# argriffing/raoteh

Hardware: AMD Instinct MI355X
Metric: site log-likelihoods/sec (batched tree pruning) (higher is better)
Workload: dtype f64; 1 GPU; c3: 61-state MG94 codon, 64-leaf balanced tree, 10000 sites/GPU, dense f64 leaf likelihood vectors; encoding=dense, sites_per_gpu=10000, sites_total=10000, states=61, leaves=64, edges=126, batches_rotated=3, reduce=none

## Files before the change

### include/raoteh_hip.h

```cpp
#ifndef RAOTEH_HIP_H
#define RAOTEH_HIP_H

#include <stdint.h>

#ifdef __cplusplus
extern "C" {
#endif

#define RT_OK                0
#define RT_ERR_INVALID      -1
#define RT_ERR_HIP          -2
#define RT_ERR_UNSUPPORTED  -3
#define RT_ERR_NOMEM        -4
#define RT_ERR_RCCL         -5
#define RT_ERR_SINGULAR     -6
#define RT_ERR_ZERO_PROB    -7

#define RT_MAX_STATES      128
#define RT_MAX_EXPECT_STATES 64
#define RT_MAX_EXPECT_STEP_STATES 128
#define RT_MAX_EXPM_STATES 128

#define RT_SITE_OK           0
#define RT_SITE_ZERO_PROB    1
// ... 73 lines not shown
            const double *subtree_probability, const double *node_to_distn_array,
            double *joint_distns);

int rt_mjp_esd_expectation_weights(rt_ctx *ctx, int64_t nnodes, int64_t n,
            int64_t nsites, const int64_t *tree_csr_indices,
            const int64_t *tree_csr_indptr, const double *esd_transitions,
            const double *root_distn, const int64_t *state_mask,
            const double *site_weights, double *edge_weights, int32_t *status);

int rt_mjp_esd_expectation_weights_obs(rt_ctx *ctx, int64_t nnodes, int64_t n,
            int64_t nsites, const int64_t *tree_csr_indices,
            const int64_t *tree_csr_indptr, const double *esd_transitions,
            const double *root_distn, int64_t nobs, const int64_t *obs_nodes, int kind,
            const void *data, const double *site_weights, double *edge_weights,
            int32_t *status);

int rt_mjp_frechet_statistics(rt_ctx *ctx, int64_t n, int64_t nedges, const double *Q,
            int64_t nq, const int64_t *q_index, const double *t, const double *W,
            double *dwell, double *trans);


int rt_model_create(rt_ctx *ctx, int64_t nnodes, int64_t n,
            const int64_t *tree_csr_indices, const int64_t *tree_csr_indptr,
            rt_model **model);
int rt_model_destroy(rt_model *model);

int rt_model_set_rates(rt_model *model, const double *Q, int64_t nq,
            const int64_t *node_q, const double *t);
int rt_model_set_rates_spectral(rt_model *model, const double *A, const double *lam,
            const double *B, const double *D, const double *t);
int rt_model_recompute_transitions(rt_model *model);
int rt_model_set_transitions(rt_model *model, const double *esd_transitions);
int rt_model_get_transitions(rt_model *model, double *esd_transitions);
int rt_model_get_expm_info(rt_model *model, int32_t *info );
int rt_model_set_root_distn(rt_model *model, const double *root_distn);

int rt_model_schedule_depth(const rt_model *model);
int rt_model_get_schedule(const rt_model *model, int32_t *ops, int64_t capacity,
            int64_t *nops);
int rt_build_schedule(int64_t nnodes, const int64_t *tree_csr_indices,
            const int64_t *tree_csr_indptr, int32_t *ops ,
            int32_t *depth);
int rt_set_option(const char *key, int64_t value);
int rt_ctx_set_option(rt_ctx *ctx, const char *key, int64_t value);
int rt_jit_source(int64_t nnodes, const int64_t *tree_csr_indices,
            const int64_t *tree_csr_indptr, int64_t n, int64_t nobs,
            const int64_t *obs_nodes, int64_t prefetch, char *buf, int64_t capacity);

int rt_sites_create(rt_model *model, int64_t nsites, int kind, int64_t nobs,
            const int64_t *obs_nodes, const void *data, rt_sites **sites);
int rt_sites_clone(rt_sites *sites, rt_sites **clone);
int rt_sites_jit_wait(rt_sites *sites);
int rt_jit_wait_all(void);
int rt_sites_destroy(rt_sites *sites);
int64_t rt_sites_device_bytes(const rt_sites *sites);
double rt_sites_jit_compile_seconds(const rt_sites *sites);
int rt_debug_jit_global(rt_sites *sites, const char *name, void *dst, int64_t bytes);
const char *rt_sites_kernel_name(const rt_sites *sites);

int rt_prune(rt_model *model, rt_sites *sites);
int rt_step(rt_model *model, rt_sites *sites, int recompute_transitions);
int rt_expect_step(rt_model *model, rt_sites *sites, int recompute_transitions,
            double *dwell, double *root_posterior, double *trans, int32_t *status);
#define RT_MAX_POSTERIOR_SETS 8
int rt_sites_posteriors(rt_model *model, rt_sites *sites, int recompute_transitions,
            int64_t n_node_sets, const uint64_t *node_sets,
// ... 136 lines not shown
```

### raoteh_amd/_lib.py

```python
from __future__ import annotations

import ctypes
import os
from ctypes import (POINTER, c_char_p, c_double, c_int, c_int32,
                    c_int64, c_ubyte, c_void_p)

__all__ = ['HipLibraryError', 'RaotehHipError', 'lib', 'check', 'LIB_PATH']

LIB_PATH = os.environ.get(
    'RAOTEH_HIP_LIB',
    os.path.join(os.path.dirname(os.path.abspath(__file__)), 'libraoteh_hip.so'))

RT_OK = 0
RT_ERR_INVALID = -1
RT_ERR_HIP = -2
RT_ERR_UNSUPPORTED = -3
RT_ERR_NOMEM = -4
RT_ERR_RCCL = -5
RT_ERR_SINGULAR = -6
RT_ERR_ZERO_PROB = -7

RT_OBS_DENSE, RT_OBS_STATE, RT_OBS_MASK = 0, 1, 2
RT_K_EXPM, RT_K_PRUNE, RT_K_REDUCE, RT_K_COMBINE = 0, 1, 2, 3
RT_SITE_ZERO_PROB = 1
# ... 53 lines not shown
    'rt_mcy_esd_get_node_to_pmap': (c_int, [c_void_p, c_int64, c_int64, c_int64,
                                            _p_i64, _p_i64, _p_f64, _p_i64,
                                            _p_f64, _p_f64]),
    'rt_mcy_esd_passes': (c_int, [c_void_p, c_int64, c_int64, c_int64,
                                  _p_i64, _p_i64, _p_f64, _p_i64,
                                  _p_f64, _p_f64]),
    'rt_mc0_esd_get_node_to_distn': (c_int, [c_void_p, c_int64, c_int64, c_int64,
                                             _p_i64, _p_i64, _p_f64, _p_f64,
                                             _p_f64, _p_f64, _p_i32]),
    'rt_mc0_esd_get_joint_endpoint_distn': (c_int, [c_void_p, c_int64, c_int64,
                                                    c_int64, _p_i64, _p_i64,
                                                    _p_f64, _p_f64, _p_f64,
                                                    _p_f64]),
    'rt_mjp_esd_expectation_weights': (c_int, [c_void_p, c_int64, c_int64, c_int64,
                                               _p_i64, _p_i64, _p_f64, _p_f64, _p_i64,
                                               _p_f64, _p_f64, _p_i32]),
    'rt_mjp_esd_expectation_weights_obs': (c_int, [c_void_p, c_int64, c_int64, c_int64,
                                                   _p_i64, _p_i64, _p_f64, _p_f64, c_int64,
                                                   _p_i64, c_int, c_void_p, _p_f64, _p_f64,
                                                   _p_i32]),
    'rt_mjp_frechet_statistics': (c_int, [c_void_p, c_int64, c_int64, _p_f64, c_int64, _p_i64,
                                          _p_f64, _p_f64, _p_f64, _p_f64]),
    'rt_model_create': (c_int, [c_void_p, c_int64, c_int64, _p_i64, _p_i64,
                                POINTER(c_void_p)]),
    'rt_model_destroy': (c_int, [c_void_p]),
    'rt_model_set_rates': (c_int, [c_void_p, _p_f64, c_int64, _p_i64, _p_f64]),
    'rt_model_set_rates_spectral': (c_int, [c_void_p, _p_f64, _p_f64, _p_f64, _p_f64, _p_f64]),
    'rt_expm_spectral': (c_int, [c_void_p, c_int64, c_int64, _p_f64, _p_f64, _p_f64, _p_f64,
                                 _p_f64, _p_f64]),
    'rt_model_recompute_transitions': (c_int, [c_void_p]),
    'rt_model_set_transitions': (c_int, [c_void_p, _p_f64]),
    'rt_model_get_transitions': (c_int, [c_void_p, _p_f64]),
    'rt_model_get_expm_info': (c_int, [c_void_p, _p_i32]),
    'rt_model_set_root_distn': (c_int, [c_void_p, _p_f64]),
    'rt_model_schedule_depth': (c_int, [c_void_p]),
    'rt_model_get_schedule': (c_int, [c_void_p, _p_i32, c_int64, _p_i64]),
    'rt_build_schedule': (c_int, [c_int64, _p_i64, _p_i64, _p_i32, _p_i32]),
    'rt_set_option': (c_int, [c_char_p, c_int64]),
    'rt_ctx_set_option': (c_int, [c_void_p, c_char_p, c_int64]),
    'rt_sites_jit_compile_seconds': (c_double, [c_void_p]),
    'rt_sites_kernel_name': (c_char_p, [c_void_p]),
    'rt_debug_jit_global': (c_int, [c_void_p, c_char_p, c_void_p, c_int64]),
    'rt_jit_source': (c_int, [c_int64, _p_i64, _p_i64, c_int64, c_int64, _p_i64, c_int64,
                              c_char_p, c_int64]),
    'rt_sites_create': (c_int, [c_void_p, c_int64, c_int, c_int64, _p_i64,
                                c_void_p, POINTER(c_void_p)]),
    'rt_sites_clone': (c_int, [c_void_p, POINTER(c_void_p)]),
    'rt_sites_jit_wait': (c_int, [c_void_p]),
    'rt_jit_wait_all': (c_int, []),
    'rt_expect_step': (c_int, [c_void_p, c_void_p, c_int, _p_f64, _p_f64, _p_f64, _p_i32]),
    'rt_sites_posteriors': (c_int, [c_void_p, c_void_p, c_int, c_int64, c_void_p, c_int64,
                                    c_void_p, c_int64, _p_i64, _p_f64, _p_f64, _p_f64, _p_i32]),
    'rt_sites_branch_expectations': (c_int, [c_void_p, c_void_p, c_int, c_int64, _p_f64, _p_f64,
                                             _p_f64, _p_i32]),
    'rt_sites_branch_profiles': (c_int, [c_void_p, c_void_p, c_int, c_int64, _p_f64, _p_f64,
                                         _p_f64, _p_i32]),
    'rt_model_get_branch_lengths': (c_int, [c_void_p, _p_f64]),
    'rt_model_nni_moves': (c_int, [c_void_p, _p_i32, c_int64, _p_i64]),
    'rt_tree_nni_moves': (c_int, [c_int64, _p_i64, _p_i64, _p_i32, c_int64, _p_i64]),
    'rt_sites_nni_scores': (c_int, [c_void_p, c_void_p, c_int, c_int64, _p_f64, _p_f64, _p_f64,
                                    _p_i32]),
    'rt_sites_placements': (c_int, [c_void_p, c_void_p, c_int, c_int64, c_int, c_void_p, c_int64,
                                    _p_f64, c_int64, _p_f64, _p_f64, _p_f64, _p_i32]),
    'rt_model_spr_moves': (c_int, [c_void_p, c_int64, _p_i32, c_int64, _p_i64]),
    'rt_tree_spr_moves': (c_int, [c_int64, _p_i64, _p_i64, c_int64, _p_i32, c_int64, _p_i64]),
    'rt_sites_spr_scores': (c_int, [c_void_p, c_void_p, c_int, c_int64, c_int64, _p_f64, _p_f64,
# ... 105 lines not shown
```

### raoteh_amd/csrc/api.hip

```cpp
#include "common.h"
#include "partition_plan.h"

#include <algorithm>
#include <atomic>
#include <functional>
#include <cmath>
#include <cstdlib>


static thread_local char g_err[512] = "";

void rt_set_error(const char *fmt, ...)
{
    va_list ap;
    va_start(ap, fmt);
    vsnprintf(g_err, sizeof(g_err), fmt, ap);
    va_end(ap);
}

extern "C" const char *rt_last_error(void) { return g_err; }
extern "C" int rt_version(void) { return 100; }

extern "C" int rt_device_count(int *count)
{
// ... 748 lines not shown
    r.nq = nq;
    return rate_sets_run_expm(m);
}

extern "C" int rt_model_recompute_transitions(rt_model *m)
{
    RT_REQUIRE(m, "null model");
    RT_REQUIRE(m->d_Q || m->spectral, "rt_model_set_rates has not been called");
    RT_HIP(hipSetDevice(m->ctx->device));
    return model_run_expm(m);
}

extern "C" int rt_model_set_transitions(rt_model *m, const double *esd)
{
    RT_REQUIRE(m && esd, "null pointer");
    RT_HIP(hipSetDevice(m->ctx->device));
    RT_HIP(hipStreamSynchronize(m->ctx->stream));
    RT_HIP(hipMemcpy(m->d_P, esd, (size_t)m->nnodes * m->n * m->n * 8,
                     hipMemcpyHostToDevice));
    m->have_P = true;
    m->rates_current = false;
    m->frag_dirty = true;
    return rt_launch_pfrag(m);
}

extern "C" int rt_model_get_transitions(rt_model *m, double *esd)
{
    RT_REQUIRE(m && esd, "null pointer");
    RT_REQUIRE(m->have_P, "the model has no transition matrices yet");
    RT_HIP(hipSetDevice(m->ctx->device));
    RT_HIP(hipStreamSynchronize(m->ctx->stream));
    RT_HIP(hipMemcpy(esd, m->d_P, (size_t)m->nnodes * m->n * m->n * 8,
                     hipMemcpyDeviceToHost));
    return RT_OK;
}

extern "C" int rt_model_get_expm_info(rt_model *m, int32_t *info)
{
    RT_REQUIRE(m && info, "null pointer");
    RT_HIP(hipSetDevice(m->ctx->device));
    RT_HIP(hipStreamSynchronize(m->ctx->stream));
    RT_HIP(hipMemcpy(info, m->d_info, (size_t)m->nnodes * 8, hipMemcpyDeviceToHost));
    for (int64_t v = 1; v < m->nnodes; ++v)
        if (info[2 * v] < 0) {
            rt_set_error("expm: the matrix of the edge above node %lld has a non-finite entry or "
                         "norm (Taylor scheme), or its Pade denominator is singular "
                         "(RAOTEH_EXPM=pade)", (long long)v);
            return RT_ERR_SINGULAR;
        }
    return RT_OK;
}

extern "C" int rt_model_set_root_distn(rt_model *m, const double *root_distn)
{
    RT_REQUIRE(m, "null model");
    RT_HIP(hipSetDevice(m->ctx->device));
    std::vector<double> w((size_t)m->n, 1.0);
    if (root_distn) w.assign(root_distn, root_distn + m->n);
    RT_HIP(hipStreamSynchronize(m->ctx->stream));
    RT_HIP(hipMemcpy(m->d_root, w.data(), m->n * 8, hipMemcpyHostToDevice));
    return RT_OK;
}

extern "C" int rt_model_schedule_depth(const rt_model *m)
{
    return m ? m->max_depth : -1;
// ... 1933 lines not shown
```

### raoteh_amd/csrc/common.h

```cpp
#pragma once

#include <hip/hip_runtime.h>
#include <hip/hip_ext.h>

#include <cstdarg>
#include <cstdint>
#include <cstdio>
#include <cstring>
#include <memory>
#include <string>
#include <type_traits>
#include <vector>

#include "../../include/raoteh_hip.h"


void rt_set_error(const char *fmt, ...);

#define RT_HIP(call)                                                          \
    do {                                                                      \
        hipError_t e_ = (call);                                               \
        if (e_ != hipSuccess) {                                               \
            rt_set_error("%s failed: %s (%s:%d)", #call,                      \
                         hipGetErrorString(e_), __FILE__, __LINE__);          \
// ... 61 lines not shown
    char name[64] = "";
};

static const int RT_TOTALS_SLOTS = 4096;

struct rt_ctx {
    int device = 0;
    hipStream_t stream = nullptr;
    int num_cus = 0;
    bool timing = false;
    int timing_period = 1;
    rt_timing_slot slots[RT_K_COUNT];
    hipEvent_t ev_start = nullptr, ev_stop = nullptr;
    double *d_totals_arena = nullptr;
    std::vector<int> totals_free;
    hipEvent_t ev_reduced = nullptr;
    hipEvent_t comm_events[8] = {};
    int comm_event_next = 0;
    unsigned char *d_scratch = nullptr;
    size_t scratch_bytes = 0;
    void *comm = nullptr;
    hipStream_t comm_stream = nullptr;
    void *rccl = nullptr;
    int opt_force_generic = -2;
    int opt_jit = -2;
    int opt_jit_block_sites = -2;
    int opt_jit_async = -2;
    int opt_rescale = -2;
    int opt_leaf_state_kernels = -2;
    struct rt_sites *pending_reduce = nullptr;
    size_t expm_attr_lds = 0;
    size_t expm_ts_attr_lds[8] = {0, 0, 0, 0, 0, 0, 0, 0};
    size_t expm_split_attr_lds = 0;
    size_t expm_w8_attr_lds[3] = {0, 0, 0};
    size_t expm_wide_attr_lds[8] = {0, 0, 0, 0, 0, 0, 0, 0};
    double *d_expm_scratch = nullptr;
    void *expect_cache = nullptr;
    size_t expm_scratch_bytes = 0;
    int live_models = 0, live_chains = 0;
};
static const int RT_OPT_UNSET = -2;

static const int RT_FAST_MAX_DEPTH = 16;

struct rt_op {
    int32_t node;
    int32_t obs;
    int32_t pop;
    int32_t dst;
};

struct rt_rate_sets {
    int64_t K = 0;
    int64_t capacity = 0;
    int64_t nq = 0, q_capacity = 0;
    uint64_t epoch = 0;
    double *d_Q = nullptr;
    int32_t *d_qidx = nullptr;
    double *d_t = nullptr;
    int32_t *d_info = nullptr;
    int32_t *d_step_of_node = nullptr;
    double *d_P = nullptr;
    double *d_Pfrag = nullptr, *d_Pquad = nullptr, *d_Pcol = nullptr;
    int64_t pcol_capacity = 0;
    int64_t P_stride = 0, frag_stride = 0, quad_stride = 0, pcol_stride = 0;
};

// ... 314 lines not shown
```

### raoteh_amd/csrc/expm.hip

```cpp
#include "common.h"

#include <algorithm>
#include "reduce.h"

#include <cstdlib>

namespace {

__constant__ double c_theta[5] = {1.495585217958292e-2, 2.539398330063230e-1,
                                  9.504178996162932e-1, 2.097847961257068e0,
                                  5.371920351148152e0};
__constant__ double c_b3[4] = {120., 60., 12., 1.};
__constant__ double c_b5[6] = {30240., 15120., 3360., 420., 30., 1.};
__constant__ double c_b7[8] = {17297280., 8648640., 1995840., 277200.,
                               25200., 1512., 56., 1.};
__constant__ double c_b9[10] = {17643225600., 8821612800., 2075673600.,
                                302702400., 30270240., 2162160., 110880.,
                                3960., 90., 1.};
__constant__ double c_b13[14] = {64764752532480000., 32382376266240000.,
                                 7771770303897600., 1187353796428800.,
                                 129060195264000., 10559470521600.,
                                 670442572800., 33522128640., 1323241920.,
                                 40840800., 960960., 16380., 182., 1.};

// ... 586 lines not shown
}

template <int NT>
__device__ __forceinline__ void wave8_tiles(int wave, int &m, int &j0, int &nc)
{
    if (NT == 4) { m = wave >> 1; j0 = 2 * (wave & 1); nc = 2; }
    else if (wave < 6) { m = wave / 3; j0 = wave - 3 * m; nc = 1; }
    else { m = 2; j0 = wave == 6 ? 0 : 2; nc = wave == 6 ? 2 : 1; }
}

template <int NT>
__device__ __forceinline__ void load_left8(const double *X, int m, double (&a)[4 * NT])
{
    constexpr int LD = 16 * NT + 1;
    const int lane = threadIdx.x & 63;
    const double *ap = X + (16 * m + (lane & 15)) * LD + (lane >> 4);
#pragma unroll
    for (int kk = 0; kk < 4 * NT; ++kk) a[kk] = ap[4 * kk];
}

template <int NT>
__device__ __forceinline__ void load_tiles8(const double *M, half_tiles &t, int m, int j0, int nc)
{
    constexpr int LD = 16 * NT + 1;
    const int lane = threadIdx.x & 63;
    const int lr = lane & 15, lq = lane >> 4;
#pragma unroll
    for (int v = 0; v < 2; ++v)
#pragma unroll
        for (int r = 0; r < 4; ++r)
            t.v[v][r] = v < nc ? M[(16 * m + 4 * r + lq) * LD + 16 * (j0 + v) + lr] : 0.0;
}

template <int NT, int NC>
__device__ __forceinline__ void mm8(const double (&a)[4 * NT], const double *Y, double *C,
                                    int m, int j0, int nc_wave, bool seed, double c0, double c1,
                                    double c2, double nd, const half_tiles *R1,
                                    const half_tiles *R2, half_tiles *out = nullptr,
                                    const double *top = nullptr, double *C2 = nullptr,
                                    bool fine = false)
{
    RT_FINE(0);
    constexpr int LD = 16 * NT + 1, KS = 4 * NT;
    const int nc = NC ? NC : nc_wave;
    const int lane = threadIdx.x & 63;
    const int lr = lane & 15, lq = lane >> 4;
    const double *bp = Y + lq * LD + 16 * j0 + lr;
    const int o1 = nc > 1 ? 16 : 0;
    double b00 = bp[0], b01 = bp[o1];
    double b10 = bp[4 * LD], b11 = bp[4 * LD + o1];
    double4_t acc[2];
#pragma unroll
    for (int v = 0; v < 2; ++v) {
        acc[v] = (double4_t){0.0, 0.0, 0.0, 0.0};
        if (seed && v < nc) {
            const int col = 16 * (j0 + v) + lr;
#pragma unroll
            for (int r = 0; r < 4; ++r) {
                const int row = 16 * m + 4 * r + lq;
                double w = c1 * R1->v[v][r];
                w = fma(c2, R2->v[v][r], w);
                if (row == col && (double)row < nd) w += c0;
                acc[v][r] = w;
            }
        }
    }
    RT_FINE(1);
#pragma unroll
    for (int kk = 0; kk < KS; ++kk) {
        const int kn = kk + 2 < KS ? kk + 2 : KS - 1;
        const double b20 = bp[4 * kn * LD], b21 = bp[4 * kn * LD + o1];
        __builtin_amdgcn_sched_barrier(0);
        acc[0] = __builtin_amdgcn_mfma_f64_16x16x4f64(a[kk], b00, acc[0], 0, 0, 0);
        if (NC != 1 && nc > 1)
            acc[1] = __builtin_amdgcn_mfma_f64_16x16x4f64(a[kk], b01, acc[1], 0, 0, 0);
        __builtin_amdgcn_sched_barrier(0);
        b00 = b10; b01 = b11;
        b10 = b20; b11 = b21;
    }
    RT_FINE(2);
    if (out) {
#pragma unroll
        for (int v = 0; v < 2; ++v)
#pragma unroll
            for (int r = 0; r < 4; ++r) out->v[v][r] = acc[v][r];
    }
    __syncthreads();
    RT_FINE(3);
#pragma unroll
    for (int v = 0; v < 2; ++v)
        if (v < nc) {
            const int col = 16 * (j0 + v) + lr;
#pragma unroll
            for (int r = 0; r < 4; ++r) {
                const int row = 16 * m + 4 * r + lq;
                C[row * LD + col] = acc[v][r];
                if (top) {
                    double w = top[1] * R1->v[v][r];
                    w = fma(top[2], R2->v[v][r], w);
                    w = fma(top[3], acc[v][r], w);
                    C2[row * LD + col] = w + ((row == col && (double)row < top[4]) ? top[0] : 0.0);
                }
            }
        }
    RT_FINE(4);
    __syncthreads();
    RT_FINE(5);
}

__device__ int rt_expm_trace_on = 0;
__device__ unsigned long long rt_expm_trace[8];
#define RT_EXPM_STAMP(k)                                                              \
    if (trace_on && blockIdx.x == (SPLIT ? 2 : 1) && threadIdx.x == 0)                \
        rt_expm_trace[k] = __builtin_readcyclecounter()

template <int NT, bool GLOBAL, bool SPLIT = false, int WAVES = 4>
__global__ void __launch_bounds__(64 * WAVES)
expm_taylor_kernel(int n, const double *__restrict__ Q, const int *__restrict__ qidx,
                   const double *__restrict__ tt, double *__restrict__ P,
                   int *__restrict__ info, const int *__restrict__ step_of_node,
                   int frag_kind, double *__restrict__ Pfrag, double *__restrict__ Pquad,
                   double *__restrict__ scratch, rt_reduce_args red)
{
    extern __shared__ __attribute__((aligned(16))) unsigned char smem[];
    if (red.partial && blockIdx.x == gridDim.x - 1) {
        rt_reduce_partials_body(red.partial, red.npartials, red.totals, red.nsites);
        return;
    }
    constexpr int RN = 16 * NT;
    constexpr int LD = RN + 1;
    constexpr int MSZ = RN * LD;
    __shared__ double colsum[RN];
    const int trace_on = rt_expm_trace_on;
    RT_EXPM_STAMP(0);
    double *B0 = GLOBAL ? scratch + (size_t)blockIdx.x * 4 * MSZ : (double *)smem;
    double *B1 = B0 + MSZ;
    double *B2 = B1 + MSZ;
    double *B3 = B2 + MSZ;

    static_assert(!SPLIT || (NT == 4 && !GLOBAL), "two workgroups per matrix: 49 <= n <= 64");
    static_assert(WAVES == 4 || (WAVES == 8 && !GLOBAL && (NT == 3 || NT == 4)),
                  "two waves per SIMD: LDS-resident, 33 <= n <= 64");
    constexpr int NTH = 64 * WAVES;
    const int b = SPLIT ? (int)(blockIdx.x >> 1) : (int)blockIdx.x;
    const int half = SPLIT ? (int)(blockIdx.x & 1) : 0;
    const int tid = threadIdx.x;
    const int nn = n * n;
    const int KSn = (n + 3) / 4, NTn = (n + 15) / 16;
    double *Pb = P + (long)b * nn;
    const int qi = qidx[b];
    const int step = step_of_node ? step_of_node[b] : -1;
    constexpr int RP0 = GLOBAL ? 1 : TPB / RN;
    constexpr int PER0 = GLOBAL ? 1 : (RN + RP0 - 1) / RP0;
    double q0[PER0];
    if (!GLOBAL) {
        const int jc = tid % RN, g = tid / RN;
#pragma unroll
        for (int u = 0; u < PER0; ++u) {
            const int i = g + u * RP0;
            q0[u] = (g < RP0 && i < n && jc < n) ? Q[i * n + jc] : 0.0;
        }
    }
    const double t_early = tt[b];
    if (qi < 0) {
        for (int e = tid; e < nn; e += NTH) Pb[e] = 0.0;
        if (info && tid == 0) { info[2 * b] = 0; info[2 * b + 1] = 0; }
        if (step >= 0 && frag_kind == 0)
            for (int e = tid; e < nn; e += NTH) Pfrag[(long)step * nn + e] = 0.0;
        if (step >= 0 && frag_kind == 1) {
            const int total = NTn * ((KSn + 1) / 2) * 128;
            for (int e = tid; e < total; e += NTH) Pfrag[(long)step * total + e] = 0.0;
            if (Pquad)
                for (int e = tid; e < KSn * KSn * 16; e += NTH)
                    Pquad[(long)step * rt_quad_stride(n) + e] = 0.0;
        }
        return;
    }
    const double *Qb = Q + (long)qi * nn;
    const double t = t_early;
    double nrm = 0.0;
    if (!GLOBAL) {
        constexpr int RP = TPB / RN;
        constexpr int PER = (RN + RP - 1) / RP;
        __shared__ double colpart[RP][RN];
        const int jc = tid % RN, g = tid / RN;
        const bool active = g < RP;
        double v[PER];
        double part = 0.0;
        if (qi > 0) {
#pragma unroll
            for (int u = 0; u < PER; ++u) {
                const int i = g + u * RP;
                q0[u] = (active && i < n && jc < n) ? Qb[i * n + jc] : 0.0;
            }
        }
#pragma unroll
        for (int u = 0; u < PER; ++u) v[u] = q0[u] * t;
#pragma unroll
        for (int u = 0; u < PER; ++u) {
            const int i = g + u * RP;
            if (active && i < RN) B0[i * LD + jc] = v[u];
            part += fabs(v[u]);
        }
        if (active) colpart[g][jc] = part;
        __syncthreads();
        if (tid < RN) {
            double sum = 0.0;
#pragma unroll
            for (int r = 0; r < RP; ++r) sum += colpart[r][tid];
            colsum[tid] = sum;
        }
        __syncthreads();
        {
            const int ln = tid & 63;
            nrm = ln < RN ? colsum[ln] : 0.0;
#pragma unroll
            for (int o = 32; o > 0; o >>= 1) nrm = fmax(nrm, __shfl_xor(nrm, o, 64));
        }
    } else {
        constexpr int PER = (MSZ + TPB - 1) / TPB;
        for (int c0 = 0; c0 < PER; c0 += 8) {
            double v[8];
#pragma unroll
            for (int u = 0; u < 8; ++u) {
                const int e = (c0 + u) * TPB + tid;
                const int i = e / LD, jx = e - i * LD;
                v[u] = (e < MSZ && i < n && jx < n) ? Qb[i * n + jx] * t : 0.0;
            }
#pragma unroll
            for (int u = 0; u < 8; ++u) {
                const int e = (c0 + u) * TPB + tid;
                if (e < MSZ) B0[e] = v[u];
            }
        }
        __syncthreads();
        for (int jx = tid; jx < RN; jx += TPB) {
            double sum = 0.0;
            for (int i = 0; i < n; ++i) sum += fabs(B0[i * LD + jx]);
            colsum[jx] = sum;
        }
        __syncthreads();
        for (int jj = 0; jj < RN; ++jj) nrm = fmax(nrm, colsum[jj]);
    }
    RT_EXPM_STAMP(1);
    if (!(nrm < 1e300)) {
        for (int e = tid; e < nn; e += NTH) Pb[e] = __builtin_nan("");
        if (info && tid == 0) { info[2 * b] = -1; info[2 * b + 1] = 0; }
        return;
    }
    int m = 15, s = 0;
    if (nrm <= c_theta_taylor[0]) m = 3;
    else if (nrm <= c_theta_taylor[1]) m = 6;
    else if (nrm <= c_theta_taylor[2]) m = 9;
    else if (nrm <= c_theta_taylor[3]) m = 12;
    else if (nrm > c_theta_taylor[4]) {
        int e;
        const double f = frexp(nrm / c_theta_taylor[4], &e);
        s = (f == 0.5) ? e - 1 : e;
        if (s < 0) s = 0;
    }
    m = __builtin_amdgcn_readfirstlane(m);
    s = __builtin_amdgcn_readfirstlane(s);
    if (info && tid == 0) { info[2 * b] = m; info[2 * b + 1] = s; }
    if (s > 0) {
        const double sc = ldexp(1.0, -s);
        for (int e = tid; e < MSZ; e += NTH) B0[e] *= sc;
        __syncthreads();
    }
    const int q = m / 3;
    RT_EXPM_STAMP(2);
    if constexpr (WAVES == 8) {
        const int wave = __builtin_amdgcn_readfirstlane(tid >> 6);
        int wm, wj, wn;
        wave8_tiles<NT>(wave, wm, wj, wn);
        constexpr int NCF = NT == 4 ? 2 : 0;
        const double nd = (double)n;
        const double tops8[5] = {c_inv_fact[3 * (q - 1)], c_inv_fact[3 * (q - 1) + 1],
                                 c_inv_fact[3 * (q - 1) + 2], c_inv_fact[m], nd};
        double left[4 * NT];
        half_tiles ra, ra2;
        load_left8<NT>(B0, wm, left);
        load_tiles8<NT>(B0, ra, wm, wj, wn);
        mm8<NT, NCF>(left, B0, B1, wm, wj, wn, false, 0.0, 0.0, 0.0, nd, nullptr, nullptr,
                     &ra2);
        mm8<NT, NCF>(left, B1, B2, wm, wj, wn, false, 0.0, 0.0, 0.0, nd, &ra, &ra2, nullptr,
                     tops8, B3);
        RT_EXPM_STAMP(3);
        RT_EXPM_STAMP(4);
        if (q >= 2) load_left8<NT>(B2, wm, left);
        if (SPLIT && s == 0) {
            if constexpr (SPLIT) {
                const int hj = 2 * half + (wave & 1);
                half_tiles ha, ha2;
                load_tiles8<NT>(B0, ha, wm, hj, 1);
                load_tiles8<NT>(B1, ha2, wm, hj, 1);
#pragma unroll
                for (int u = 3; u >= 0; --u)
                    if (u <= q - 2)
                        mm8<NT, 1>(left, B3, B3, wm, hj, 1, true, c_inv_fact[3 * u],
                                   c_inv_fact[3 * u + 1], c_inv_fact[3 * u + 2], nd, &ha, &ha2,
                                   nullptr, nullptr, nullptr,
                                   trace_on && blockIdx.x == 2 && u == 0);
            }
        } else {
            for (int jj = q - 2; jj >= 0; --jj)
                mm8<NT, NCF>(left, B3, B3, wm, wj, wn, true, c_inv_fact[3 * jj],
                             c_inv_fact[3 * jj + 1], c_inv_fact[3 * jj + 2], nd, &ra, &ra2);
        }
        RT_EXPM_STAMP(5);
        for (int r = 0; r < s; ++r) {
            load_left8<NT>(B3, wm, left);
            mm8<NT, NCF>(left, B3, B3, wm, wj, wn, false, 0.0, 0.0, 0.0, nd, nullptr, nullptr);
        }
    } else {
        lane_tiles<NT> ra, ra2;
        load_tiles<NT>(B0, ra);
        mm_blocked<NT>(B0, B0, B1, nullptr, nullptr, nullptr, nullptr, nullptr, &ra2);
        __shared__ double tops[5];
        {
            const int base = 3 * (q - 1);
            if (tid == 0) {
                tops[0] = c_inv_fact[base];
                tops[1] = c_inv_fact[base + 1];
                tops[2] = c_inv_fact[base + 2];
                tops[3] = c_inv_fact[m];
                tops[4] = (double)n;
            }
            __syncthreads();
        }
        mm_blocked<NT>(B0, B1, B2, nullptr, nullptr, nullptr, &ra, &ra2, nullptr, tops, B3);
        RT_EXPM_STAMP(3);
        RT_EXPM_STAMP(4);
        __shared__ double cfs_all[5][4];
        if (tid < 20) cfs_all[tid >> 2][tid & 3] = (tid & 3) == 3 ? (double)n
                                                                 : c_inv_fact[3 * (tid >> 2) + (tid & 3)];
        __syncthreads();
        if (SPLIT && s == 0) {
            if constexpr (SPLIT) {
                half_tiles ha, ha2;
                load_half_tiles(B0, ha, half);
                load_half_tiles(B1, ha2, half);
                double hc[4][3];
#pragma unroll
                for (int u = 0; u < 4; ++u)
#pragma unroll
                    for (int e = 0; e < 3; ++e) hc[u][e] = c_inv_fact[3 * u + e];
                const double nd = (double)n;
#pragma unroll
                for (int u = 3; u >= 0; --u)
                    if (u <= q - 2)
                        mm_half(B2, B3, B3, hc[u][0], hc[u][1], hc[u][2], nd, ha, ha2, half,
                                trace_on && blockIdx.x == 2 && u == 0);
            }
        } else {
            for (int jj = q - 2; jj >= 0; --jj)
                mm_blocked<NT>(B2, B3, B3, cfs_all[jj], B0, B1, &ra, &ra2);
        }
        RT_EXPM_STAMP(5);
        for (int r = 0; r < s; ++r) mm_blocked<NT>(B3, B3, B3, nullptr, nullptr, nullptr);
    }
    RT_EXPM_STAMP(6);

    const double *Xb = B3;
    if constexpr (SPLIT) {
        const int jc = 32 * half + (tid & 31), g = tid >> 5;
        if (jc < n)
            for (int i = g; i < n; i += NTH / 32) Pb[i * n + jc] = Xb[i * LD + jc];
        if (step >= 0 && frag_kind == 1) {
            const int KP = (KSn + 1) / 2;
            const int total = NTn * KP * 128;
            for (int blk = tid >> 7; blk < NTn * 4; blk += NTH >> 7) {
                const int mm = blk >> 2, qq = 4 * half + (blk & 3);
                if (qq < KP) {
                    const int e = (mm * KP + qq) * 128 + (tid & 127);
                    const int e2 = e & 1;
                    const int ln = (e >> 1) & 63;
                    const int row = 16 * mm + (ln & 15);
                    const int col = 4 * (2 * qq + e2) + (ln >> 4);
                    Pfrag[(long)step * total + e] = (col < RN) ? Xb[row * LD + col] : 0.0;
                }
            }
        }
        RT_EXPM_STAMP(7);
        return;
    }
    if (!GLOBAL) {
        constexpr int RP = NTH / RN;
        const int jc = tid % RN, g = tid / RN;
        if (g < RP && jc < n)
            for (int i = g; i < n; i += RP) Pb[i * n + jc] = Xb[i * LD + jc];
    } else {
        for (int e = tid; e < nn; e += TPB) {
            const int i = e / n, j = e - i * n;
            Pb[e] = Xb[i * LD + j];
        }
    }
// ... 320 lines not shown
        const char *wv = getenv("RAOTEH_EXPM_WIDE");
        if (global && !(wv && atoi(wv) == 0) && !d_Pquad) {
            bool split2 = 2 * vcount + extra <= (int64_t)std::max(2, ctx->num_cus);
            if (const char *v = getenv("RAOTEH_EXPM_SPLIT")) split2 = atoi(v) != 0;
            const size_t wgs = (size_t)count * (split2 ? 2 : 1);
            const size_t need = wgs * ((nt + 1) / 2) * 4 * nt * 256 * 8;
            if (need > ctx->expm_scratch_bytes) {
                RT_HIP(hipStreamSynchronize(ctx->stream));
                hipFree(ctx->d_expm_scratch);
                ctx->d_expm_scratch = nullptr;
                ctx->expm_scratch_bytes = 0;
                RT_HIP(hipMalloc((void **)&ctx->d_expm_scratch, need));
                ctx->expm_scratch_bytes = need;
            }
            RT_TRY(rt_expm_wide_launch(ctx, nt, split2, wgs + extra, n, d_Q, d_qidx, d_t, d_P, d_info,
                                       d_step_of_node, frag_kind, d_Pfrag, red));
            return RT_OK;
        }
        hipEvent_t ev = nullptr;
        rt_time_begin(ctx, RT_K_EXPM, global ? "expm_taylor_ps_mfma_global" : "expm_taylor_ps_mfma",
                      &ev);
#define RT_TAYLOR(NTV, GL)                                                                      \
        do {                                                                                    \
            if (lds_t > ctx->expm_ts_attr_lds[NTV - 1]) {                                       \
                RT_HIP(hipFuncSetAttribute((const void *)expm_taylor_kernel<NTV, GL>,           \
                                           hipFuncAttributeMaxDynamicSharedMemorySize,          \
                                           (int)lds_t));                                        \
                ctx->expm_ts_attr_lds[NTV - 1] = lds_t;                                         \
            }                                                                                   \
            RT_LAUNCH_TIMED(ctx, (expm_taylor_kernel<NTV, GL>), dim3((unsigned)count + extra),  \
                            dim3(TPB), lds_t, (int)n, d_Q, d_qidx, d_t, d_P, d_info,            \
                            d_step_of_node, frag_kind, d_Pfrag, d_Pquad, scratch, red);         \
        } while (0)
#define RT_TAYLOR8(NTV, SP, SLOT)                                                               \
        do {                                                                                    \
            if (lds_t > ctx->expm_w8_attr_lds[SLOT]) {                                          \
                RT_HIP(hipFuncSetAttribute((const void *)expm_taylor_kernel<NTV, false, SP, 8>, \
                                           hipFuncAttributeMaxDynamicSharedMemorySize,          \
                                           (int)lds_t));                                        \
                ctx->expm_w8_attr_lds[SLOT] = lds_t;                                            \
            }                                                                                   \
            RT_LAUNCH_TIMED(ctx, (expm_taylor_kernel<NTV, false, SP, 8>),                       \
                            dim3((SP ? 2u : 1u) * (unsigned)count + extra), dim3(512), lds_t,   \
                            (int)n, d_Q, d_qidx, d_t, d_P, d_info, d_step_of_node, frag_kind,   \
                            d_Pfrag, d_Pquad, scratch, red);                                    \
        } while (0)
        const char *wv8 = getenv("RAOTEH_EXPM_WAVES");
        const bool waves8 = (nt == 3 || nt == 4) && !(wv8 && atoi(wv8) == 4);
        bool split2 = nt == 4 && 2 * vcount + extra <= (int64_t)std::max(2, ctx->num_cus) && !d_Pquad;
        if (const char *v = getenv("RAOTEH_EXPM_SPLIT")) split2 = nt == 4 && !d_Pquad && atoi(v) != 0;
        if (split2 && waves8) {
            snprintf(ctx->slots[RT_K_EXPM].name, sizeof(ctx->slots[RT_K_EXPM].name),
                     "expm_taylor_ps_mfma_split2");
            RT_TAYLOR8(4, true, 2);
        } else if (split2) {
            if (lds_t > ctx->expm_split_attr_lds) {
                RT_HIP(hipFuncSetAttribute((const void *)expm_taylor_kernel<4, false, true>,
                                           hipFuncAttributeMaxDynamicSharedMemorySize, (int)lds_t));
                ctx->expm_split_attr_lds = lds_t;
            }
            snprintf(ctx->slots[RT_K_EXPM].name, sizeof(ctx->slots[RT_K_EXPM].name),
                     "expm_taylor_ps_mfma_split2");
            RT_LAUNCH_TIMED(ctx, (expm_taylor_kernel<4, false, true>),
                            dim3(2u * (unsigned)count + extra), dim3(TPB), lds_t, (int)n, d_Q, d_qidx,
                            d_t, d_P, d_info, d_step_of_node, frag_kind, d_Pfrag, d_Pquad, scratch,
                            red);
        } else
        switch (nt) {
        case 1: RT_TAYLOR(1, false); break;
        case 2: RT_TAYLOR(2, false); break;
        case 3: if (waves8) RT_TAYLOR8(3, false, 0); else RT_TAYLOR(3, false); break;
        case 4: if (waves8) RT_TAYLOR8(4, false, 1); else RT_TAYLOR(4, false); break;
        case 5: RT_TAYLOR(5, true); break;
        case 6: RT_TAYLOR(6, true); break;
        case 7: RT_TAYLOR(7, true); break;
        default: RT_TAYLOR(8, true); break;
        }
#undef RT_TAYLOR
#undef RT_TAYLOR8
        RT_HIP(hipGetLastError());
        if (getenv("RAOTEH_EXPM_TRACE")) {
            static int armed = 0;
            unsigned long long tr[8];
            RT_HIP(hipStreamSynchronize(ctx->stream));
            if (armed) {
                RT_HIP(hipMemcpyFromSymbol(tr, HIP_SYMBOL(rt_expm_trace), sizeof tr));
                unsigned long long fn[8];
                RT_HIP(hipMemcpyFromSymbol(fn, HIP_SYMBOL(rt_expm_fine), sizeof fn));
                fprintf(stderr, "[raoteh_amd] last Horner half product: seed + first operands %llu, k loop "
                        "%llu, barrier %llu, write-back %llu, barrier %llu\n", fn[1] - fn[0],
                        fn[2] - fn[1], fn[3] - fn[2], fn[4] - fn[3], fn[5] - fn[4]);
                fprintf(stderr, "[raoteh_amd] expm trace (clocks, workgroup 1): load + norm %llu, order %llu, "
                        "A^2 A^3 %llu, block %llu, Horner %llu, squarings %llu, store %llu; total %llu\n",
                        tr[1] - tr[0], tr[2] - tr[1], tr[3] - tr[2], tr[4] - tr[3], tr[5] - tr[4],
                        tr[6] - tr[5], tr[7] - tr[6], tr[7] - tr[0]);
            }
            const int on = 1;
            RT_HIP(hipMemcpyToSymbol(HIP_SYMBOL(rt_expm_trace_on), &on, sizeof on));
            armed = 1;
        }
        rt_time_end(ctx, RT_K_EXPM, ev);
        return RT_OK;
    }
    hipEvent_t ev = nullptr;
    rt_time_begin(ctx, RT_K_EXPM, "expm_mfma_regsolve", &ev);
    RT_LAUNCH_TIMED(ctx, expm_kernel, dim3((unsigned)count + extra), dim3(TPB), lds,
                       (int)n, d_Q, d_qidx, d_t, d_P, d_info, d_step_of_node, frag_kind,
                       d_Pfrag, d_Pquad, red);
    RT_HIP(hipGetLastError());
    rt_time_end(ctx, RT_K_EXPM, ev);
    return RT_OK;
}
// ... 1 lines not shown
```

### raoteh_amd/device.py

```python
from __future__ import annotations

import atexit
import collections
import ctypes
import weakref
from ctypes import byref, c_char_p, c_double, c_int, c_int32, c_int64, c_void_p

import numpy as np

from . import _lib
from ._tree import TreeArrays

__all__ = ['check_rate_sets', 'check_site_sets', 'Context', 'get_context', 'TreeModel', 'SiteBatch', 'device_count', 'Posteriors',
           'states_to_mask', 'BranchExpectations', 'check_branch_coefs', 'SampledStates', 'SampledMappings',
           'MapStates']

_shutting_down = []
atexit.register(_shutting_down.append, True)

_KINDS = {'dense': _lib.RT_OBS_DENSE, 'state': _lib.RT_OBS_STATE,
          'mask': _lib.RT_OBS_MASK}


def _f64(a):
# ... 763 lines not shown
        A, lam, B = _f64(A), _f64(lam), _f64(B)
        n = self.nstates
        if A.shape != (n, n) or B.shape != (n, n) or lam.shape != (n,):
            raise ValueError('expected the array to be square')
        D = None if D is None else _f64(D)
        if D is not None and D.shape != (n,):
            raise ValueError('D must have one entry per state')
        if t is None:
            t = self.tree.branch_lengths()
        t = _f64(t)
        if t.shape != (self.tree.nnodes,):
            raise ValueError('t must have one entry per node')
        _lib.check(_lib.lib().rt_model_set_rates_spectral(
            self._h, _ptr(A, c_double), _ptr(lam, c_double), _ptr(B, c_double),
            None if D is None else _ptr(D, c_double), _ptr(t, c_double)))
        self._rates = None

    def recompute_transitions(self):
        _lib.check(_lib.lib().rt_model_recompute_transitions(self._h))

    def set_transitions(self, esd):
        esd = _f64(esd)
        if esd.shape != (self.tree.nnodes, self.nstates, self.nstates):
            raise ValueError('esd_transitions has the wrong shape')
        _lib.check(_lib.lib().rt_model_set_transitions(self._h,
                                                       _ptr(esd, c_double)))

    def get_transitions(self):
        esd = np.empty((self.tree.nnodes, self.nstates, self.nstates))
        _lib.check(_lib.lib().rt_model_get_transitions(self._h,
                                                       _ptr(esd, c_double)))
        return esd

    def expm_info(self):
        info = np.zeros((self.tree.nnodes, 2), dtype=np.int32)
        _lib.check(_lib.lib().rt_model_get_expm_info(self._h,
                                                     _ptr(info, c_int32)))
        return info

    def set_root_distn(self, root_distn=None):
        if root_distn is None:
            _lib.check(_lib.lib().rt_model_set_root_distn(self._h, None))
            self._root_w = None
            return
        w = _f64(root_distn)
        if w.shape != (self.nstates,):
            raise ValueError('root shape mismatch: %s %s' % (
                (self.nstates,), w.shape))
        _lib.check(_lib.lib().rt_model_set_root_distn(self._h,
                                                      _ptr(w, c_double)))
        self._root_w = w.copy()

    def upload_sites(self, obs_nodes, data, kind='dense', site_sets=None, nsets=None):
        code = _KINDS[kind]
        idx = _i64([self.tree.node_to_index[v] for v in obs_nodes])
        if kind == 'dense':
            data = _f64(data)
            ok = data.ndim == 3 and data.shape[2] == self.nstates
        elif kind == 'state':
            data = _as_uint8_states(data, self.nstates)
            ok = data.ndim == 2
        else:
            data = np.ascontiguousarray(data, dtype=np.uint64)
            words = (self.nstates + 63) // 64
            ok = (data.ndim == 2 and words == 1) or (data.ndim == 3 and data.shape[2] == words)
        if not ok or data.shape[1] != len(idx):
# ... 539 lines not shown
```

Before: 55.23 million sites/s.

## Add lean eight-wave expm form overlapping norm/order with first product and ping-pong buffers

Adds a LEAN variant of the eight-wave Taylor expm kernel. One wave computes the 1-norm and Taylor order while the others start the first matrix product speculatively, redoing it only when scaling is needed. The Horner and squaring steps now ping-pong between two buffers, which lets mm8 skip the aliasing barrier. It is on by default unless RAOTEH_EXPM_SERIAL=0, and a fragment read-back API is added alongside. The prune-throughput metric only benefits if the expm kernel falls within the timed region.

```diff
diff --git a/include/raoteh_hip.h b/include/raoteh_hip.h
--- a/include/raoteh_hip.h
+++ b/include/raoteh_hip.h
@@ -129,6 +129,7 @@
 int rt_model_recompute_transitions(rt_model *model);
 int rt_model_set_transitions(rt_model *model, const double *esd_transitions);
 int rt_model_get_transitions(rt_model *model, double *esd_transitions);
+int rt_model_get_fragments(rt_model *model, double *frags, int64_t *ndoubles);
 int rt_model_get_expm_info(rt_model *model, int32_t *info );
 int rt_model_set_root_distn(rt_model *model, const double *root_distn);
 
diff --git a/raoteh_amd/_lib.py b/raoteh_amd/_lib.py
--- a/raoteh_amd/_lib.py
+++ b/raoteh_amd/_lib.py
@@ -109,6 +109,7 @@
     'rt_model_set_transitions': (c_int, [c_void_p, _p_f64]),
     'rt_model_get_transitions': (c_int, [c_void_p, _p_f64]),
     'rt_model_get_expm_info': (c_int, [c_void_p, _p_i32]),
+    'rt_model_get_fragments': (c_int, [c_void_p, _p_f64, _p_i64]),
     'rt_model_set_root_distn': (c_int, [c_void_p, _p_f64]),
     'rt_model_schedule_depth': (c_int, [c_void_p]),
     'rt_model_get_schedule': (c_int, [c_void_p, _p_i32, c_int64, _p_i64]),
diff --git a/raoteh_amd/csrc/api.hip b/raoteh_amd/csrc/api.hip
--- a/raoteh_amd/csrc/api.hip
+++ b/raoteh_amd/csrc/api.hip
@@ -804,6 +804,22 @@
     RT_HIP(hipStreamSynchronize(m->ctx->stream));
     RT_HIP(hipMemcpy(esd, m->d_P, (size_t)m->nnodes * m->n * m->n * 8,
                      hipMemcpyDeviceToHost));
+    return RT_OK;
+}
+
+extern "C" int rt_model_get_fragments(rt_model *m, double *frags, int64_t *ndoubles)
+{
+    RT_REQUIRE(m && ndoubles, "null pointer");
+    if (!frags) {
+        *ndoubles = pfrag_doubles(m);
+        return RT_OK;
+    }
+    RT_REQUIRE(m->have_P, "the model has no transition matrices yet");
+    RT_REQUIRE(*ndoubles >= 0 && *ndoubles <= pfrag_doubles(m), "the image has %lld doubles",
+               (long long)pfrag_doubles(m));
+    RT_HIP(hipSetDevice(m->ctx->device));
+    RT_HIP(hipStreamSynchronize(m->ctx->stream));
+    RT_HIP(hipMemcpy(frags, m->d_Pfrag, (size_t)*ndoubles * 8, hipMemcpyDeviceToHost));
     return RT_OK;
 }
 
diff --git a/raoteh_amd/csrc/common.h b/raoteh_amd/csrc/common.h
--- a/raoteh_amd/csrc/common.h
+++ b/raoteh_amd/csrc/common.h
@@ -117,7 +117,7 @@
     size_t expm_attr_lds = 0;
     size_t expm_ts_attr_lds[8] = {0, 0, 0, 0, 0, 0, 0, 0};
     size_t expm_split_attr_lds = 0;
-    size_t expm_w8_attr_lds[3] = {0, 0, 0};
+    size_t expm_w8_attr_lds[6] = {0, 0, 0, 0, 0, 0};
     size_t expm_wide_attr_lds[8] = {0, 0, 0, 0, 0, 0, 0, 0};
     double *d_expm_scratch = nullptr;
     void *expect_cache = nullptr;
diff --git a/raoteh_amd/csrc/expm.hip b/raoteh_amd/csrc/expm.hip
--- a/raoteh_amd/csrc/expm.hip
+++ b/raoteh_amd/csrc/expm.hip
@@ -642,7 +642,7 @@
             t.v[v][r] = v < nc ? M[(16 * m + 4 * r + lq) * LD + 16 * (j0 + v) + lr] : 0.0;
 }
 
-template <int NT, int NC>
+template <int NT, int NC, bool ALIAS = true>
 __device__ __forceinline__ void mm8(const double (&a)[4 * NT], const double *Y, double *C,
                                     int m, int j0, int nc_wave, bool seed, double c0, double c1,
                                     double c2, double nd, const half_tiles *R1,
@@ -695,7 +695,7 @@
 #pragma unroll
             for (int r = 0; r < 4; ++r) out->v[v][r] = acc[v][r];
     }
-    __syncthreads();
+    if (ALIAS) __syncthreads();
     RT_FINE(3);
 #pragma unroll
     for (int v = 0; v < 2; ++v)
@@ -718,13 +718,29 @@
     RT_FINE(5);
 }
 
+__device__ __forceinline__ void taylor_order(double nrm, int &m, int &s)
+{
+    m = 15;
+    s = 0;
+    if (nrm <= c_theta_taylor[0]) m = 3;
+    else if (nrm <= c_theta_taylor[1]) m = 6;
+    else if (nrm <= c_theta_taylor[2]) m = 9;
+    else if (nrm <= c_theta_taylor[3]) m = 12;
+    else if (nrm > c_theta_taylor[4]) {
+        int e;
+        const double f = frexp(nrm / c_theta_taylor[4], &e);
+        s = (f == 0.5) ? e - 1 : e;
+        if (s < 0) s = 0;
+    }
+}
+
 __device__ int rt_expm_trace_on = 0;
 __device__ unsigned long long rt_expm_trace[8];
 #define RT_EXPM_STAMP(k)                                                              \
     if (trace_on && blockIdx.x == (SPLIT ? 2 : 1) && threadIdx.x == 0)                \
         rt_expm_trace[k] = __builtin_readcyclecounter()
 
-template <int NT, bool GLOBAL, bool SPLIT = false, int WAVES = 4>
+template <int NT, bool GLOBAL, bool SPLIT = false, int WAVES = 4, bool LEAN = false>
 __global__ void __launch_bounds__(64 * WAVES)
 expm_taylor_kernel(int n, const double *__restrict__ Q, const int *__restrict__ qidx,
                    const double *__restrict__ tt, double *__restrict__ P,
@@ -751,6 +767,8 @@
     static_assert(!SPLIT || (NT == 4 && !GLOBAL), "two workgroups per matrix: 49 <= n <= 64");
     static_assert(WAVES == 4 || (WAVES == 8 && !GLOBAL && (NT == 3 || NT == 4)),
                   "two waves per SIMD: LDS-resident, 33 <= n <= 64");
+    static_assert(!LEAN || WAVES == 8, "the form with fewer barriers is an eight-wave form");
+    __shared__ int order_lds[2];
     constexpr int NTH = 64 * WAVES;
     const int b = SPLIT ? (int)(blockIdx.x >> 1) : (int)blockIdx.x;
     const int half = SPLIT ? (int)(blockIdx.x & 1) : 0;
@@ -814,6 +832,20 @@
         }
         if (active) colpart[g][jc] = part;
         __syncthreads();
+        if constexpr (LEAN) {
+            if (tid >> 6 == 7) {
+                const int ln = tid & 63;
+                double sum = 0.0;
+#pragma unroll
+                for (int r = 0; r < RP; ++r) sum += colpart[r][ln < RN ? ln : 0];
+                nrm = ln < RN ? sum : 0.0;
+#pragma unroll
+                for (int o = 32; o > 0; o >>= 1) nrm = fmax(nrm, __shfl_xor(nrm, o, 64));
+                int m7 = -1, s7 = 0;
+                if (nrm < 1e300) taylor_order(nrm, m7, s7);
+                if (ln == 0) { order_lds[0] = m7; order_lds[1] = s7; }
+            }
+        } else {
         if (tid < RN) {
             double sum = 0.0;
 #pragma unroll
@@ -826,6 +858,7 @@
             nrm = ln < RN ? colsum[ln] : 0.0;
 #pragma unroll
             for (int o = 32; o > 0; o >>= 1) nrm = fmax(nrm, __shfl_xor(nrm, o, 64));
+        }
         }
     } else {
         constexpr int PER = (MSZ + TPB - 1) / TPB;
@@ -853,22 +886,14 @@
         for (int jj = 0; jj < RN; ++jj) nrm = fmax(nrm, colsum[jj]);
     }
     RT_EXPM_STAMP(1);
+    int m = 15, s = 0;
+    if constexpr (!LEAN) {
     if (!(nrm < 1e300)) {
         for (int e = tid; e < nn; e += NTH) Pb[e] = __builtin_nan("");
         if (info && tid == 0) { info[2 * b] = -1; info[2 * b + 1] = 0; }
         return;
     }
-    int m = 15, s = 0;
-    if (nrm <= c_theta_taylor[0]) m = 3;
-    else if (nrm <= c_theta_taylor[1]) m = 6;
-    else if (nrm <= c_theta_taylor[2]) m = 9;
-    else if (nrm <= c_theta_taylor[3]) m = 12;
-    else if (nrm > c_theta_taylor[4]) {
-        int e;
-        const double f = frexp(nrm / c_theta_taylor[4], &e);
-        s = (f == 0.5) ? e - 1 : e;
-        if (s < 0) s = 0;
-    }
+    taylor_order(nrm, m, s);
     m = __builtin_amdgcn_readfirstlane(m);
     s = __builtin_amdgcn_readfirstlane(s);
     if (info && tid == 0) { info[2 * b] = m; info[2 * b + 1] = s; }
@@ -877,7 +902,9 @@
         for (int e = tid; e < MSZ; e += NTH) B0[e] *= sc;
         __syncthreads();
     }
-    const int q = m / 3;
+    }
+    int q = m / 3;
+    double *last = B3;
     RT_EXPM_STAMP(2);
     if constexpr (WAVES == 8) {
         const int wave = __builtin_amdgcn_readfirstlane(tid >> 6);
@@ -885,19 +912,52 @@
         wave8_tiles<NT>(wave, wm, wj, wn);
         constexpr int NCF = NT == 4 ? 2 : 0;
         const double nd = (double)n;
-        const double tops8[5] = {c_inv_fact[3 * (q - 1)], c_inv_fact[3 * (q - 1) + 1],
-                                 c_inv_fact[3 * (q - 1) + 2], c_inv_fact[m], nd};
+        double tops8[5];
+        if constexpr (!LEAN) {
+            tops8[0] = c_inv_fact[3 * (q - 1)];
+            tops8[1] = c_inv_fact[3 * (q - 1) + 1];
+            tops8[2] = c_inv_fact[3 * (q - 1) + 2];
+            tops8[3] = c_inv_fact[m];
+            tops8[4] = nd;
+        }
+        constexpr bool AL = !LEAN;
         double left[4 * NT];
         half_tiles ra, ra2;
         load_left8<NT>(B0, wm, left);
         load_tiles8<NT>(B0, ra, wm, wj, wn);
-        mm8<NT, NCF>(left, B0, B1, wm, wj, wn, false, 0.0, 0.0, 0.0, nd, nullptr, nullptr,
-                     &ra2);
-        mm8<NT, NCF>(left, B1, B2, wm, wj, wn, false, 0.0, 0.0, 0.0, nd, &ra, &ra2, nullptr,
-                     tops8, B3);
+        mm8<NT, NCF, AL>(left, B0, B1, wm, wj, wn, false, 0.0, 0.0, 0.0, nd, nullptr, nullptr,
+                         &ra2);
+        if constexpr (LEAN) {
+            m = __builtin_amdgcn_readfirstlane(order_lds[0]);
+            s = __builtin_amdgcn_readfirstlane(order_lds[1]);
+            if (m < 0) {
+                for (int e = tid; e < nn; e += NTH) Pb[e] = __builtin_nan("");
+                if (info && tid == 0) { info[2 * b] = -1; info[2 * b + 1] = 0; }
+                return;
+            }
+            if (info && tid == 0) { info[2 * b] = m; info[2 * b + 1] = s; }
+            if (s > 0) {
+                const double sc = ldexp(1.0, -s);
+                for (int e = tid; e < MSZ; e += NTH) B0[e] *= sc;
+                __syncthreads();
+                load_left8<NT>(B0, wm, left);
+                load_tiles8<NT>(B0, ra, wm, wj, wn);
+                mm8<NT, NCF, false>(left, B0, B1, wm, wj, wn, false, 0.0, 0.0, 0.0, nd, nullptr,
+                                    nullptr, &ra2);
+            }
+            q = m / 3;
+            tops8[0] = c_inv_fact[3 * (q - 1)];
+            tops8[1] = c_inv_fact[3 * (q - 1) + 1];
+            tops8[2] = c_inv_fact[3 * (q - 1) + 2];
+            tops8[3] = c_inv_fact[m];
+            tops8[4] = nd;
+        }
+        mm8<NT, NCF, AL>(left, B1, B2, wm, wj, wn, false, 0.0, 0.0, 0.0, nd, &ra, &ra2, nullptr,
+                         tops8, B3);
         RT_EXPM_STAMP(3);
         RT_EXPM_STAMP(4);
         if (q >= 2) load_left8<NT>(B2, wm, left);
+        double *cur = B3, *nxt = LEAN ? B0 : B3;
         if (SPLIT && s == 0) {
             if constexpr (SPLIT) {
                 const int hj = 2 * half + (wave & 1);
@@ -906,22 +966,28 @@
                 load_tiles8<NT>(B1, ha2, wm, hj, 1);
 #pragma unroll
                 for (int u = 3; u >= 0; --u)
-                    if (u <= q - 2)
-                        mm8<NT, 1>(left, B3, B3, wm, hj, 1, true, c_inv_fact[3 * u],
-                                   c_inv_fact[3 * u + 1], c_inv_fact[3 * u + 2], nd, &ha, &ha2,
-                                   nullptr, nullptr, nullptr,
-                                   trace_on && blockIdx.x == 2 && u == 0);
+                    if (u <= q - 2) {
+                        mm8<NT, 1, AL>(left, cur, nxt, wm, hj, 1, true, c_inv_fact[3 * u],
+                                       c_inv_fact[3 * u + 1], c_inv_fact[3 * u + 2], nd, &ha, &ha2,
+                                       nullptr, nullptr, nullptr,
+                                       trace_on && blockIdx.x == 2 && u == 0);
+                        double *was = cur; cur = nxt; nxt = was;
+                    }
             }
         } else {
-            for (int jj = q - 2; jj >= 0; --jj)
-                mm8<NT, NCF>(left, B3, B3, wm, wj, wn, true, c_inv_fact[3 * jj],
-                             c_inv_fact[3 * jj + 1], c_inv_fact[3 * jj + 2], nd, &ra, &ra2);
+            for (int jj = q - 2; jj >= 0; --jj) {
+                mm8<NT, NCF, AL>(left, cur, nxt, wm, wj, wn, true, c_inv_fact[3 * jj],
+                                 c_inv_fact[3 * jj + 1], c_inv_fact[3 * jj + 2], nd, &ra, &ra2);
+                double *was = cur; cur = nxt; nxt = was;
+            }
         }
         RT_EXPM_STAMP(5);
         for (int r = 0; r < s; ++r) {
-            load_left8<NT>(B3, wm, left);
-            mm8<NT, NCF>(left, B3, B3, wm, wj, wn, false, 0.0, 0.0, 0.0, nd, nullptr, nullptr);
-        }
+            load_left8<NT>(cur, wm, left);
+            mm8<NT, NCF, AL>(left, cur, nxt, wm, wj, wn, false, 0.0, 0.0, 0.0, nd, nullptr, nullptr);
+            double *was = cur; cur = nxt; nxt = was;
+        }
+        last = cur;
     } else {
         lane_tiles<NT> ra, ra2;
         load_tiles<NT>(B0, ra);
@@ -971,7 +1037,7 @@
     }
     RT_EXPM_STAMP(6);
 
-    const double *Xb = B3;
+    const double *Xb = last;
     if constexpr (SPLIT) {
         const int jc = 32 * half + (tid & 31), g = tid >> 5;
         if (jc < n)
@@ -1358,21 +1424,28 @@
                             dim3(TPB), lds_t, (int)n, d_Q, d_qidx, d_t, d_P, d_info,            \
                             d_step_of_node, frag_kind, d_Pfrag, d_Pquad, scratch, red);         \
         } while (0)
-#define RT_TAYLOR8(NTV, SP, SLOT)                                                               \
+#define RT_TAYLOR8_FORM(NTV, SP, SLOT, LN)                                                      \
         do {                                                                                    \
-            if (lds_t > ctx->expm_w8_attr_lds[SLOT]) {                                          \
-                RT_HIP(hipFuncSetAttribute((const void *)expm_taylor_kernel<NTV, false, SP, 8>, \
-                                           hipFuncAttributeMaxDynamicSharedMemorySize,          \
-                                           (int)lds_t));                                        \
-                ctx->expm_w8_attr_lds[SLOT] = lds_t;                                            \
+            if (lds_t > ctx->expm_w8_attr_lds[SLOT + (LN ? 3 : 0)]) {                           \
+                RT_HIP(hipFuncSetAttribute(                                                     \
+                    (const void *)expm_taylor_kernel<NTV, false, SP, 8, LN>,                    \
+                    hipFuncAttributeMaxDynamicSharedMemorySize, (int)lds_t));                   \
+                ctx->expm_w8_attr_lds[SLOT + (LN ? 3 : 0)] = lds_t;                             \
             }                                                                                   \
-            RT_LAUNCH_TIMED(ctx, (expm_taylor_kernel<NTV, false, SP, 8>),                       \
+            RT_LAUNCH_TIMED(ctx, (expm_taylor_kernel<NTV, false, SP, 8, LN>),                   \
                             dim3((SP ? 2u : 1u) * (unsigned)count + extra), dim3(512), lds_t,   \
                             (int)n, d_Q, d_qidx, d_t, d_P, d_info, d_step_of_node, frag_kind,   \
                             d_Pfrag, d_Pquad, scratch, red);                                    \
         } while (0)
+#define RT_TAYLOR8(NTV, SP, SLOT)                                                               \
+        do {                                                                                    \
+            if (lean8) RT_TAYLOR8_FORM(NTV, SP, SLOT, true);                                    \
+            else RT_TAYLOR8_FORM(NTV, SP, SLOT, false);                                         \
+        } while (0)
         const char *wv8 = getenv("RAOTEH_EXPM_WAVES");
         const bool waves8 = (nt == 3 || nt == 4) && !(wv8 && atoi(wv8) == 4);
+        const char *sv8 = getenv("RAOTEH_EXPM_SERIAL");
+        const bool lean8 = !(sv8 && sv8[0] && atoi(sv8) == 0);
         bool split2 = nt == 4 && 2 * vcount + extra <= (int64_t)std::max(2, ctx->num_cus) && !d_Pquad;
         if (const char *v = getenv("RAOTEH_EXPM_SPLIT")) split2 = nt == 4 && !d_Pquad && atoi(v) != 0;
         if (split2 && waves8) {
@@ -1404,6 +1477,7 @@
         }
 #undef RT_TAYLOR
 #undef RT_TAYLOR8
+#undef RT_TAYLOR8_FORM
         RT_HIP(hipGetLastError());
         if (getenv("RAOTEH_EXPM_TRACE")) {
             static int armed = 0;
diff --git a/raoteh_amd/device.py b/raoteh_amd/device.py
--- a/raoteh_amd/device.py
+++ b/raoteh_amd/device.py
@@ -819,6 +819,14 @@
                                                        _ptr(esd, c_double)))
         return esd
 
+    def get_fragments(self):
+        count = np.zeros(1, dtype=np.int64)
+        _lib.check(_lib.lib().rt_model_get_fragments(self._h, None, _ptr(count, c_int64)))
+        frags = np.empty(int(count[0]))
+        _lib.check(_lib.lib().rt_model_get_fragments(self._h, _ptr(frags, c_double),
+                                                     _ptr(count, c_int64)))
+        return frags
+
     def expm_info(self):
         info = np.zeros((self.tree.nnodes, 2), dtype=np.int32)
         _lib.check(_lib.lib().rt_model_get_expm_info(self._h,
```

New measurement: 55.36 million sites/s, median of 3. About the same (+0.2%).
